# JoeyYoung/adapcc

Hardware: NVIDIA B200
Metric: gpt2_small_ddp_train_tokens_per_sec (higher is better)
Workload: dtype bf16; 1 GPU; model=gpt2-small-double-heads (12L d768 h12 ctx1024 vocab50262, 124476673 params), global_batch=4, per_gpu_batch=4, candidates=2, seq_len=1024, parallelism=dp1, engine=graph, algo=auto, optimizer=adamw+clip1.0 (fused), grad_dtype=bf16, zero_copy_grads=False, buckets=6, zero1=False, lm_rows=all, lm_chunk_rows=8192, relay_control=False

## Files before the change

### adapcc_b200/csrc/ops_norm.cu

```cuda
#include <cuda_bf16.h>

#include <algorithm>

#include "common.h"
#include "device_prims.cuh"

namespace adapcc {

constexpr int kLnWarps = 8;

__device__ __forceinline__ float warp_sum(float v) {
#pragma unroll
  for (int o = 16; o > 0; o >>= 1) v += __shfl_xor_sync(0xffffffffu, v, o);
  return v;
}

template <int VPL, bool RES>
__global__ void __launch_bounds__(kLnWarps * 32, VPL <= 3 ? 3 : 2)
ln_fwd_kernel(const __nv_bfloat16* __restrict__ x, const __nv_bfloat16* __restrict__ res,
              const __nv_bfloat16* __restrict__ gamma, const __nv_bfloat16* __restrict__ beta,
              __nv_bfloat16* __restrict__ sum_out, __nv_bfloat16* __restrict__ y, float* __restrict__ mean,
              float* __restrict__ rstd, int rows, float eps) {
  constexpr int D = VPL * 256;
  const int lane = threadIdx.x & 31, warp = threadIdx.x >> 5;
  uint4 gp[VPL], bp[VPL];
#pragma unroll
  for (int v = 0; v < VPL; ++v) {
    gp[v] = reinterpret_cast<const uint4*>(gamma)[lane + 32 * v];
    bp[v] = reinterpret_cast<const uint4*>(beta)[lane + 32 * v];
  }
  for (int r = blockIdx.x * kLnWarps + warp; r < rows; r += gridDim.x * kLnWarps) {
    const uint4* xr = reinterpret_cast<const uint4*>(x + (size_t)r * D);
    float f[VPL][8];
    float s = 0.f;
#pragma unroll
    for (int v = 0; v < VPL; ++v) {
      unpack<__nv_bfloat16>(ld16(xr + lane + 32 * v), f[v]);
      if constexpr (RES) {
        float fr[8];
        unpack<__nv_bfloat16>(ld16(reinterpret_cast<const uint4*>(res + (size_t)r * D) + lane + 32 * v), fr);
#pragma unroll
        for (int i = 0; i < 8; ++i) f[v][i] += fr[i];
        const uint4 packed = pack<__nv_bfloat16>(f[v]);
        st16(reinterpret_cast<uint4*>(sum_out + (size_t)r * D) + lane + 32 * v, packed);
        unpack<__nv_bfloat16>(packed, f[v]);
      }
#pragma unroll
      for (int i = 0; i < 8; ++i) s += f[v][i];
    }
    const float mu = warp_sum(s) * (1.f / D);
    float q = 0.f;
#pragma unroll
    for (int v = 0; v < VPL; ++v)
#pragma unroll
      for (int i = 0; i < 8; ++i) { const float d = f[v][i] - mu; q += d * d; }
    const float rs = rsqrtf(warp_sum(q) * (1.f / D) + eps);
    uint4* yr = reinterpret_cast<uint4*>(y + (size_t)r * D);
#pragma unroll
    for (int v = 0; v < VPL; ++v) {
      float o[8], g[8], b[8];
      unpack<__nv_bfloat16>(gp[v], g);
      unpack<__nv_bfloat16>(bp[v], b);
#pragma unroll
      for (int i = 0; i < 8; ++i) o[i] = (f[v][i] - mu) * rs * g[i] + b[i];
      st16(yr + lane + 32 * v, pack<__nv_bfloat16>(o));
    }
    if (lane == 0) { mean[r] = mu; rstd[r] = rs; }
  }
}

template <int VPL, bool RES>
__global__ void __launch_bounds__(kLnWarps * 32, VPL <= 3 ? 2 : 1)
ln_bwd_kernel(const __nv_bfloat16* __restrict__ dy, const __nv_bfloat16* __restrict__ x,
              const __nv_bfloat16* __restrict__ gamma, const float* __restrict__ mean, const float* __restrict__ rstd,
              const __nv_bfloat16* __restrict__ dres, __nv_bfloat16* __restrict__ dx,
              float* __restrict__ part_dgamma, float* __restrict__ part_dbeta, int rows) {
  constexpr int D = VPL * 256;
  const int lane = threadIdx.x & 31, warp = threadIdx.x >> 5;
  uint4 gp[VPL];
  float dg[VPL][8], db[VPL][8];
#pragma unroll
  for (int v = 0; v < VPL; ++v) {
    gp[v] = reinterpret_cast<const uint4*>(gamma)[lane + 32 * v];
#pragma unroll
    for (int i = 0; i < 8; ++i) dg[v][i] = db[v][i] = 0.f;
  }
  for (int r = blockIdx.x * kLnWarps + warp; r < rows; r += gridDim.x * kLnWarps) {
    const uint4* xr = reinterpret_cast<const uint4*>(x + (size_t)r * D);
    const uint4* dr = reinterpret_cast<const uint4*>(dy + (size_t)r * D);
    const float mu = mean[r], rs = rstd[r];
    float xh[VPL][8], gy[VPL][8];
    float c1 = 0.f, c2 = 0.f;
#pragma unroll
    for (int v = 0; v < VPL; ++v) {
      float fx[8], fd[8], g[8];
      unpack<__nv_bfloat16>(ld16(xr + lane + 32 * v), fx);
      unpack<__nv_bfloat16>(ld16(dr + lane + 32 * v), fd);
      unpack<__nv_bfloat16>(gp[v], g);
#pragma unroll
      for (int i = 0; i < 8; ++i) {
        xh[v][i] = (fx[i] - mu) * rs;
        gy[v][i] = fd[i] * g[i];
        c1 += gy[v][i];
        c2 += gy[v][i] * xh[v][i];
        dg[v][i] += fd[i] * xh[v][i];
        db[v][i] += fd[i];
      }
    }
    c1 = warp_sum(c1) * (1.f / D);
    c2 = warp_sum(c2) * (1.f / D);
    uint4* ox = reinterpret_cast<uint4*>(dx + (size_t)r * D);
#pragma unroll
    for (int v = 0; v < VPL; ++v) {
      float o[8];
#pragma unroll
      for (int i = 0; i < 8; ++i) o[i] = rs * (gy[v][i] - c1 - xh[v][i] * c2);
      if constexpr (RES) {
        float fr[8];
        unpack<__nv_bfloat16>(ld16(reinterpret_cast<const uint4*>(dres + (size_t)r * D) + lane + 32 * v), fr);
#pragma unroll
        for (int i = 0; i < 8; ++i) o[i] += fr[i];
      }
      st16(ox + lane + 32 * v, pack<__nv_bfloat16>(o));
    }
  }
  __shared__ float sm[kLnWarps][D];
#pragma unroll
  for (int pass = 0; pass < 2; ++pass) {
#pragma unroll
    for (int v = 0; v < VPL; ++v)
#pragma unroll
      for (int i = 0; i < 8; ++i) sm[warp][(lane + 32 * v) * 8 + i] = pass == 0 ? dg[v][i] : db[v][i];
    __syncthreads();
    float* out = (pass == 0 ? part_dgamma : part_dbeta) + (size_t)blockIdx.x * D;
    for (int c = threadIdx.x; c < D; c += blockDim.x) {
      float s = 0.f;
#pragma unroll
      for (int w = 0; w < kLnWarps; ++w) s += sm[w][c];
      out[c] = s;
    }
    __syncthreads();
  }
}

template <typename O>
__global__ void __launch_bounds__(1024)
colsum_finalize_kernel(const float* __restrict__ part, int nparts, int cols, O* __restrict__ out) {
  __shared__ float sm[32][33];
  const int c = blockIdx.x * 32 + threadIdx.x;
  float s = 0.f;
  if (c < cols)
    for (int p = threadIdx.y; p < nparts; p += 32) s += part[(size_t)p * cols + c];
  sm[threadIdx.y][threadIdx.x] = s;
  __syncthreads();
  if (threadIdx.y == 0 && c < cols) {
    float t = 0.f;
#pragma unroll
    for (int r = 0; r < 32; ++r) t += sm[r][threadIdx.x];
    out[c] = from_float<O>(t);
  }
}

template <typename O>
__global__ void __launch_bounds__(1024)
colsum_finalize_pair_kernel(const float* __restrict__ part_a, const float* __restrict__ part_b, int nparts, int cols,
                            O* __restrict__ out_a, O* __restrict__ out_b) {
  __shared__ float sm[32][33];
  const float* part = blockIdx.y == 0 ? part_a : part_b;
  O* out = blockIdx.y == 0 ? out_a : out_b;
  const int c = blockIdx.x * 32 + threadIdx.x;
  float s = 0.f;
  if (c < cols)
    for (int p = threadIdx.y; p < nparts; p += 32) s += part[(size_t)p * cols + c];
  sm[threadIdx.y][threadIdx.x] = s;
  __syncthreads();
  if (threadIdx.y == 0 && c < cols) {
    float t = 0.f;
#pragma unroll
    for (int r = 0; r < 32; ++r) t += sm[r][threadIdx.x];
    out[c] = from_float<O>(t);
  }
}

__global__ void __launch_bounds__(256)
colsum_partial_kernel(const __nv_bfloat16* __restrict__ a, int rows, int cols, float* __restrict__ part) {
  const int vcol = blockIdx.x * 32 + threadIdx.x;
  const int nvec = cols / 8;
  float acc[8];
#pragma unroll
  for (int i = 0; i < 8; ++i) acc[i] = 0.f;
  if (vcol < nvec) {
    for (int r = blockIdx.y * 8 + threadIdx.y; r < rows; r += gridDim.y * 8) {
      float f[8];
      unpack<__nv_bfloat16>(ld16(reinterpret_cast<const uint4*>(a + (size_t)r * cols) + vcol), f);
#pragma unroll
      for (int i = 0; i < 8; ++i) acc[i] += f[i];
    }
  }
  __shared__ float sm[8][32][8];
#pragma unroll
  for (int i = 0; i < 8; ++i) sm[threadIdx.y][threadIdx.x][i] = acc[i];
  __syncthreads();
  if (threadIdx.y == 0 && vcol < nvec) {
#pragma unroll
    for (int i = 0; i < 8; ++i) {
      float s = 0.f;
#pragma unroll
      for (int w = 0; w < 8; ++w) s += sm[w][threadIdx.x][i];
      part[(size_t)blockIdx.y * cols + vcol * 8 + i] = s;
    }
  }
}

}

using namespace adapcc;

extern "C" {

static int ln_grid(int rows, int per_sm) {
  const int groups = std::max(1, (rows + kLnWarps - 1) / kLnWarps);
  const int cap = 148 * per_sm;
  const int iters = (groups + cap - 1) / cap;
  return (groups + iters - 1) / iters;
}
static int ln_fwd_ctas_per_sm(int d) { return d <= 768 ? 3 : 2; }
static int ln_bwd_ctas_per_sm(int d) { return d <= 768 ? 2 : 1; }
int adapcc_ln_partials(int rows) { return ln_grid(rows, 2); }

static int ln_fwd_launch(const void* x, const void* res, const void* gamma, const void* beta, void* sum_out, void* y,
                         float* mean, float* rstd, int rows, int d, float eps, void* stream) {
  cudaStream_t s = (cudaStream_t)stream;
  if (rows <= 0) return 0;
  const int grid = ln_grid(rows, ln_fwd_ctas_per_sm(d));
#define LN_FWD(V)                                                                                                  \
  do {                                                                                                             \
    if (res)                                                                                                       \
      ln_fwd_kernel<V, true><<<grid, kLnWarps * 32, 0, s>>>((const __nv_bfloat16*)x, (const __nv_bfloat16*)res,    \
          (const __nv_bfloat16*)gamma, (const __nv_bfloat16*)beta, (__nv_bfloat16*)sum_out, (__nv_bfloat16*)y,     \
          mean, rstd, rows, eps);                                                                                  \
    else                                                                                                           \
      ln_fwd_kernel<V, false><<<grid, kLnWarps * 32, 0, s>>>((const __nv_bfloat16*)x, nullptr,                     \
          (const __nv_bfloat16*)gamma, (const __nv_bfloat16*)beta, nullptr, (__nv_bfloat16*)y, mean, rstd, rows,   \
          eps);                                                                                                    \
  } while (0)
  switch (d) {
    case 256: LN_FWD(1); break;
    case 512: LN_FWD(2); break;
    case 768: LN_FWD(3); break;
    case 1024: LN_FWD(4); break;
    default: set_error("ln_fwd: unsupported width %d (256/512/768/1024)", d); return -1;
  }
#undef LN_FWD
  CUDA_TRY(cudaGetLastError());
  count_launch();
  return 0;
}

int adapcc_ln_fwd(const void* x, const void* gamma, const void* beta, void* y, float* mean, float* rstd, int rows,
                  int d, float eps, void* stream) {
  return ln_fwd_launch(x, nullptr, gamma, beta, nullptr, y, mean, rstd, rows, d, eps, stream);
}

int adapcc_add_ln_fwd(const void* x, const void* res, const void* gamma, const void* beta, void* sum_out, void* y,
                      float* mean, float* rstd, int rows, int d, float eps, void* stream) {
  if (!res || !sum_out) { set_error("add_ln_fwd: res and sum_out are required"); return -1; }
  return ln_fwd_launch(x, res, gamma, beta, sum_out, y, mean, rstd, rows, d, eps, stream);
}

static int ln_bwd_launch(const void* dy, const void* x, const void* gamma, const float* mean, const float* rstd,
                         const void* dres, void* dx, void* dgamma, void* dbeta, float* part, int rows, int d,
                         void* stream) {
  cudaStream_t s = (cudaStream_t)stream;
  if (rows <= 0) return 0;
  const int grid = ln_grid(rows, ln_bwd_ctas_per_sm(d));
  float* pg = part;
  float* pb = part + (size_t)grid * d;
#define LN_BWD(V)                                                                                                  \
  do {                                                                                                             \
    if (dres)                                                                                                      \
      ln_bwd_kernel<V, true><<<grid, kLnWarps * 32, 0, s>>>((const __nv_bfloat16*)dy, (const __nv_bfloat16*)x,     \
          (const __nv_bfloat16*)gamma, mean, rstd, (const __nv_bfloat16*)dres, (__nv_bfloat16*)dx, pg, pb, rows);  \
    else                                                                                                           \
      ln_bwd_kernel<V, false><<<grid, kLnWarps * 32, 0, s>>>((const __nv_bfloat16*)dy, (const __nv_bfloat16*)x,    \
          (const __nv_bfloat16*)gamma, mean, rstd, nullptr, (__nv_bfloat16*)dx, pg, pb, rows);                     \
  } while (0)
  switch (d) {
    case 256: LN_BWD(1); break;
    case 512: LN_BWD(2); break;
    case 768: LN_BWD(3); break;
    case 1024: LN_BWD(4); break;
    default: set_error("ln_bwd: unsupported width %d (256/512/768/1024)", d); return -1;
  }
#undef LN_BWD
  CUDA_TRY(cudaGetLastError());
  colsum_finalize_pair_kernel<__nv_bfloat16><<<dim3((d + 31) / 32, 2), dim3(32, 32), 0, s>>>(
      pg, pb, grid, d, (__nv_bfloat16*)dgamma, (__nv_bfloat16*)dbeta);
  CUDA_TRY(cudaGetLastError());
  count_launch(2);
  return 0;
}

int adapcc_ln_bwd(const void* dy, const void* x, const void* gamma, const float* mean, const float* rstd, void* dx,
                  void* dgamma, void* dbeta, float* part, int rows, int d, void* stream) {
  return ln_bwd_launch(dy, x, gamma, mean, rstd, nullptr, dx, dgamma, dbeta, part, rows, d, stream);
}

int adapcc_add_ln_bwd(const void* dy, const void* x, const void* gamma, const float* mean, const float* rstd,
                      const void* dres, void* dx, void* dgamma, void* dbeta, float* part, int rows, int d,
                      void* stream) {
  return ln_bwd_launch(dy, x, gamma, mean, rstd, dres, dx, dgamma, dbeta, part, rows, d, stream);
}

int adapcc_colsum_splits(int rows) { return std::max(1, std::min(64, rows / 64)); }

int adapcc_colsum(const void* a, int rows, int cols, void* out, float* part, void* stream) {
  cudaStream_t s = (cudaStream_t)stream;
  if (cols % 8 != 0) { set_error("colsum: cols must be a multiple of 8"); return -1; }
  if (rows <= 0) return 0;
  const int splits = adapcc_colsum_splits(rows);
  dim3 grid((cols / 8 + 31) / 32, splits), block(32, 8);
  colsum_partial_kernel<<<grid, block, 0, s>>>((const __nv_bfloat16*)a, rows, cols, part);
  colsum_finalize_kernel<__nv_bfloat16><<<(cols + 31) / 32, dim3(32, 32), 0, s>>>(part, splits, cols, (__nv_bfloat16*)out);
  CUDA_TRY(cudaGetLastError());
  count_launch(2);
  return 0;
}

}
```

### adapcc_b200/models/gpt2.py

```python
from __future__ import annotations

import math
import os
from dataclasses import dataclass
from typing import Optional, Tuple

import torch
import torch.nn as nn
import torch.nn.functional as F

from ..ops.layers import FusedLayerNorm, FusedLinear


@dataclass
class GPT2Config:

    vocab_size: int = 50257 + 5
    n_positions: int = 1024
    n_embd: int = 768
    n_layer: int = 12
    n_head: int = 12
    layer_norm_epsilon: float = 1e-5
    initializer_range: float = 0.02
    lm_chunk_rows: int = 8192

    @classmethod
    def tiny(cls) -> "GPT2Config":
        return cls(vocab_size=512, n_positions=64, n_embd=64, n_layer=2, n_head=4, lm_chunk_rows=64)


class Block(nn.Module):

    def __init__(self, cfg: GPT2Config):
        super().__init__()
        d = cfg.n_embd
        self.n_head = cfg.n_head
        self.ln_1 = FusedLayerNorm(d, eps=cfg.layer_norm_epsilon)
        self.c_attn = FusedLinear(d, 3 * d)
        self.c_proj = FusedLinear(d, d)
        self.ln_2 = FusedLayerNorm(d, eps=cfg.layer_norm_epsilon)
        self.c_fc = FusedLinear(d, 4 * d)
        self.c_proj2 = FusedLinear(4 * d, d)
        self.tc_mlp = int(os.environ.get("ADAPCC_TCGEN05_MLP", "2") or 0)

    def _mlp(self, h: torch.Tensor) -> torch.Tensor:
        if self.tc_mlp and h.is_cuda and h.dtype == torch.bfloat16 and torch.is_grad_enabled():
            from ..ops.gemm import linear_gelu, mlp_gelu, supported
            if supported(h, self.c_fc.weight):
                if self.tc_mlp >= 2 and self.c_fc.weight.shape[0] % 64 == 0:
                    return mlp_gelu(h, self.c_fc.weight, self.c_fc.bias, self.c_proj2.weight, self.c_proj2.bias)
                return self.c_proj2(linear_gelu(h, self.c_fc.weight, self.c_fc.bias))
        return self.c_proj2(F.gelu(self.c_fc(h), approximate="tanh"))

    def _attn(self, h: torch.Tensor) -> torch.Tensor:
        B, T, D = h.shape
        q, k, v = (t.view(B, T, self.n_head, D // self.n_head).transpose(1, 2) for t in self.c_attn(h).split(D, dim=-1))
        a = F.scaled_dot_product_attention(q, k, v, is_causal=True)
        return self.c_proj(a.transpose(1, 2).reshape(B, T, D))

    def forward_deferred(self, x: torch.Tensor, delta: Optional[torch.Tensor]):
        if delta is None:
            h = self.ln_1(x)
        else:
            x, h = self.ln_1.forward_add(x, delta)
        x, h = self.ln_2.forward_add(x, self._attn(h))
        return x, self._mlp(h)

    def forward(self, x: torch.Tensor) -> torch.Tensor:
        x = x + self._attn(self.ln_1(x))
        return x + self._mlp(self.ln_2(x))


def use_sink(p) -> bool:
    from ..ops.layers import _sink
    return p.is_cuda and _sink(p) is not None


class _ChunkedLMLoss(torch.autograd.Function):

    @staticmethod
    def forward(ctx, h, weight, labels, chunk, vocab, scale=None):
        n = h.shape[0]
        use_kernel = h.is_cuda and h.dtype == torch.bfloat16 and weight.shape[0] % 8 == 0
        grad_h = torch.empty_like(h)
        grad_w = None
        total = torch.zeros((), dtype=torch.float32, device=h.device)
        direct = False
        if use_kernel:
            from ..ops import fused_ce_
            from ..ops.layers import _sink
            direct = (scale is not None and _sink(weight) is not None and weight.grad.dtype == h.dtype
                      and ctx.needs_input_grad[1])
        for s in range(0, n, chunk):
            hs = h[s:s + chunk]
            ls = labels[s:s + chunk]
            logits = hs @ weight.t()
            if use_kernel:
                total += fused_ce_(logits, ls, vocab, grad_scale=scale).sum()
                g = logits
            else:
                lf = logits.float()
                lf[:, vocab:] = float("-inf")
                valid = (ls >= 0)
                lse = torch.logsumexp(lf, dim=-1)
                tgt = lf.gather(1, ls.clamp(min=0).unsqueeze(1)).squeeze(1)
                total += ((lse - tgt) * valid).sum()
                p = torch.softmax(lf, dim=-1)
                p.scatter_add_(1, ls.clamp(min=0).unsqueeze(1), -torch.ones_like(p[:, :1]))
                g = p * valid.unsqueeze(1)
                if scale is not None:
                    g = g * scale
                g = g.to(h.dtype)
            torch.mm(g, weight, out=grad_h[s:s + chunk])
            if direct:
                if s == 0:
                    torch.mm(g.t(), hs, out=weight.grad)
                else:
                    weight.grad.addmm_(g.t(), hs)
            elif grad_w is None:
                grad_w = g.t() @ hs
            else:
                grad_w.addmm_(g.t(), hs)
        if scale is not None:
            total = total * scale.reshape(())
        ctx.direct, ctx.weight = direct, weight
        if direct:
            ctx.save_for_backward(grad_h)
        else:
            if grad_w is None:
                grad_w = torch.zeros_like(weight)
            ctx.save_for_backward(grad_h, grad_w)
        return total

    @staticmethod
    def backward(ctx, g):
        if ctx.direct:
            return ctx.saved_tensors[0], None, None, None, None, None
        grad_h, grad_w = ctx.saved_tensors
        gw = grad_w * g.to(grad_w.dtype)
        if use_sink(ctx.weight):
            ctx.weight.grad.add_(gw)
            gw = None
        return grad_h * g.to(grad_h.dtype), gw, None, None, None, None


class GPT2DoubleHeads(nn.Module):

    def __init__(self, cfg: Optional[GPT2Config] = None):
        super().__init__()
        self.cfg = cfg = cfg or GPT2Config()
        self.padded_vocab = (cfg.vocab_size + 63) // 64 * 64
        self.wte = nn.Embedding(self.padded_vocab, cfg.n_embd)
        self.wpe = nn.Embedding(cfg.n_positions, cfg.n_embd)
        self.h = nn.ModuleList([Block(cfg) for _ in range(cfg.n_layer)])
        self.ln_f = FusedLayerNorm(cfg.n_embd, eps=cfg.layer_norm_epsilon)
        self.mc_head = nn.Linear(cfg.n_embd, 1)
        self.lm_row_capacity = 0
        self.fuse_add_ln = os.environ.get("ADAPCC_FUSE_ADD_LN", "1") == "1"
        self.fused_embed = os.environ.get("ADAPCC_FUSED_EMBED", "1") != "0"
        if self.fused_embed:
            self.wte.weight._adapcc_embed_table = True
            self.wpe.weight._adapcc_embed_table = True
        self._pos_cache = {}
        self.apply(self._init)
        for blk in self.h:
            for lin in (blk.c_proj, blk.c_proj2):
                nn.init.normal_(lin.weight, std=cfg.initializer_range / math.sqrt(2 * cfg.n_layer))

    def _init(self, m):
        if isinstance(m, (nn.Linear, nn.Embedding)):
            nn.init.normal_(m.weight, std=self.cfg.initializer_range)
            if isinstance(m, nn.Linear) and m.bias is not None:
                nn.init.zeros_(m.bias)

    def num_parameters(self) -> int:
        return sum(p.numel() for p in self.parameters())

    def hidden(self, input_ids: torch.Tensor, token_type_ids: Optional[torch.Tensor]) -> torch.Tensor:
        N, T = input_ids.shape
        if (self.fused_embed and input_ids.is_cuda and self.wte.weight.dtype == torch.bfloat16
                and self.wpe.weight.dtype == torch.bfloat16):
            from ..ops import fused_embedding_sum
            key = (N, T, input_ids.device)
            pos = self._pos_cache.get(key)
            if pos is None:
                pos = self._pos_cache[key] = torch.arange(T, device=input_ids.device).repeat(N)
            lookups = [(0, input_ids), (1, pos)] + ([(0, token_type_ids)] if token_type_ids is not None else [])
            x = fused_embedding_sum([self.wte.weight, self.wpe.weight], lookups).view(N, T, -1)
        else:
            pos = torch.arange(T, device=input_ids.device)
            x = self.wte(input_ids) + self.wpe(pos)[None]
            if token_type_ids is not None:
                x = x + self.wte(token_type_ids)
        if self.fuse_add_ln:
            delta = None
            for blk in self.h:
                x, delta = blk.forward_deferred(x, delta)
            return self.ln_f.forward_add(x, delta)[1]
        for blk in self.h:
            x = blk(x)
        return self.ln_f(x)

    def forward(self, input_ids, token_type_ids=None, mc_token_ids=None, lm_labels=None, mc_labels=None,
                lm_coef: float = 1.0, mc_coef: float = 1.0) -> Tuple[torch.Tensor, torch.Tensor, torch.Tensor]:
        B, C, T = input_ids.shape
        ids = input_ids.reshape(B * C, T)
        tt = token_type_ids.reshape(B * C, T) if token_type_ids is not None else None
        h = self.hidden(ids, tt)
        zero = torch.zeros((), dtype=torch.float32, device=h.device)
        lm_loss, mc_loss = zero, zero
        if lm_labels is not None:
            labels = lm_labels.reshape(B * C, T)
            shift_h = h[:, :-1].reshape(-1, h.shape[-1])
            shift_l = labels[:, 1:].reshape(-1)
            n_valid = (shift_l >= 0).sum()
            cap = int(self.lm_row_capacity)
            compact = 0 < cap < shift_l.numel()
            if compact:
                order = torch.argsort((shift_l < 0).to(torch.int8), stable=True)[:cap]
                shift_h = shift_h.index_select(0, order)
                shift_l = shift_l.index_select(0, order)
            scale = (lm_coef / n_valid.clamp(min=1).to(torch.float32)).reshape(1)
            lm_term = _ChunkedLMLoss.apply(shift_h, self.wte.weight, shift_l, self.cfg.lm_chunk_rows,
                                           self.cfg.vocab_size, scale)
            lm_loss = lm_term / lm_coef if lm_coef != 0 else lm_term
            if compact:
                lm_loss = torch.where(n_valid > cap, torch.full_like(lm_loss, float("nan")), lm_loss)
                lm_term = torch.where(n_valid > cap, torch.full_like(lm_term, float("nan")), lm_term)
        if mc_token_ids is not None and mc_labels is not None:
            idx = mc_token_ids.reshape(B * C, 1, 1).expand(-1, 1, h.shape[-1])
            cls_h = h.gather(1, idx).squeeze(1)
            mc_logits = self.mc_head(cls_h).view(B, C).float()
            mc_loss = F.cross_entropy(mc_logits, mc_labels)
        loss = (lm_term if lm_labels is not None else zero) + mc_coef * mc_loss
        return loss, lm_loss, mc_loss


@torch.no_grad()
def sample_sequence(model: "GPT2DoubleHeads", input_ids: torch.Tensor, token_type_ids: Optional[torch.Tensor] = None,
                    max_new_tokens: int = 20, temperature: float = 0.7, top_k: int = 0, top_p: float = 0.9,
                    eos_token: Optional[int] = None, reply_type: Optional[int] = None,
                    generator: Optional[torch.Generator] = None) -> torch.Tensor:
    ids = input_ids.clone()
    tt = token_type_ids.clone() if token_type_ids is not None else None
    vocab = model.cfg.vocab_size
    for _ in range(max_new_tokens):
        window = slice(max(0, ids.shape[1] - model.cfg.n_positions), None)
        h = model.hidden(ids[:, window], tt[:, window] if tt is not None else None)
        logits = (h[:, -1].float() @ model.wte.weight.float().t())[:, :vocab] / max(temperature, 1e-6)
        if top_k > 0:
            kth = torch.topk(logits, min(top_k, vocab)).values[:, -1:]
            logits = logits.masked_fill(logits < kth, float("-inf"))
        if 0.0 < top_p < 1.0:
            srt, idx = torch.sort(logits, descending=True)
            cum = torch.softmax(srt, -1).cumsum(-1)
            drop = cum > top_p
            drop[:, 1:] = drop[:, :-1].clone()
            drop[:, 0] = False
            logits = logits.masked_fill(torch.zeros_like(drop).scatter(1, idx, drop), float("-inf"))
        nxt = torch.multinomial(torch.softmax(logits, -1), 1, generator=generator)
        ids = torch.cat([ids, nxt], 1)
        if tt is not None:
            tt = torch.cat([tt, torch.full_like(nxt, reply_type if reply_type is not None else int(tt[0, -1]))], 1)
        if eos_token is not None and int(nxt) == eos_token:
            break
    return ids[:, input_ids.shape[1]:]


def lm_rows_needed(lm_labels: torch.Tensor, multiple: int = 256) -> int:
    n = int((lm_labels[..., 1:] >= 0).sum())
    return max(multiple, (n + multiple - 1) // multiple * multiple)


def synthetic_batch(batch: int, candidates: int, seq_len: int, vocab: int, device="cpu", seed: int = 0,
                    pin: bool = False):
    g = torch.Generator().manual_seed(seed)
    ids = torch.randint(0, vocab, (batch, candidates, seq_len), generator=g)
    tt = torch.randint(vocab - 5, vocab - 3, (batch, candidates, seq_len), generator=g)
    labels = torch.full((batch, candidates, seq_len), -100, dtype=torch.long)
    reply = max(1, seq_len // 4)
    labels[:, -1, -reply:] = ids[:, -1, -reply:]
    mc_token_ids = torch.full((batch, candidates), seq_len - 1, dtype=torch.long)
    mc_labels = torch.full((batch,), candidates - 1, dtype=torch.long)
    out = {"input_ids": ids, "token_type_ids": tt, "lm_labels": labels, "mc_token_ids": mc_token_ids,
           "mc_labels": mc_labels}
    if pin and torch.cuda.is_available():
        out = {k: v.pin_memory() for k, v in out.items()}
    if device != "cpu":
        out = {k: v.to(device, non_blocking=True) for k, v in out.items()}
    return out
```

### adapcc_b200/ops/gemm.py

```python
from __future__ import annotations

import os
from ctypes import c_int, c_void_p
from typing import Optional, Tuple

import torch

from ..runtime.native import NativeError, last_error, load_library

_bound = False
ACT = {"none": 0, "gelu": 1, "dgelu": 2, "residual": 3}


def _lib():
    global _bound
    lib = load_library()
    if not _bound:
        lib.adapcc_gemm_bias_act_v.argtypes = [c_void_p] * 5 + [c_int] * 5 + [c_void_p]
        lib.adapcc_gemm_pp.argtypes = [c_void_p] * 6 + [c_int] * 4 + [c_void_p]
        _bound = True
    return lib


def supported(x: torch.Tensor, weight: torch.Tensor) -> bool:
    return (x.is_cuda and x.dtype == torch.bfloat16 and weight.dtype == torch.bfloat16
            and weight.shape[1] % 64 == 0 and weight.shape[0] % 128 == 0)


def default_variant() -> int:
    return int(os.environ.get("ADAPCC_TCGEN05_VARIANT", "3"))


def linear_act(x: torch.Tensor, weight: torch.Tensor, bias: Optional[torch.Tensor], act: str = "gelu",
               save_pre: bool = False, variant: Optional[int] = None,
               aux: Optional[torch.Tensor] = None,
               colsum: Optional[torch.Tensor] = None) -> Tuple[torch.Tensor, Optional[torch.Tensor]]:
    if not supported(x, weight):
        raise NativeError("linear_act: needs bf16 CUDA tensors with K % 64 == 0 and N % 128 == 0")
    n, k = weight.shape
    x2 = x.reshape(-1, k).contiguous()
    w = weight.contiguous()
    m = x2.shape[0]
    code = ACT[act]
    out = torch.empty(m, n, dtype=torch.bfloat16, device=x.device)
    v_req = default_variant() if variant is None else int(variant)
    if v_req == 3 and n % 256 == 0 and code <= 2:
        if code == 2:
            if aux is None or aux.numel() != m * n or aux.dtype != torch.bfloat16:
                raise NativeError("linear_act(dgelu): aux must be a bf16 tensor with the result's shape")
            pre = aux.reshape(m, n).contiguous()
        else:
            pre = torch.empty_like(out) if save_pre else None
        if colsum is not None and (code != 2 or colsum.dtype != torch.float32 or colsum.numel() != n):
            raise NativeError("linear_act: colsum is an fp32 [N] accumulator of the dgelu mode")
        b = bias.contiguous() if bias is not None else None
        rc = _lib().adapcc_gemm_pp(c_void_p(x2.data_ptr()), c_void_p(w.data_ptr()),
                                   c_void_p(b.data_ptr() if b is not None else 0), c_void_p(out.data_ptr()),
                                   c_void_p(pre.data_ptr() if pre is not None else 0),
                                   c_void_p(colsum.data_ptr() if colsum is not None else 0), m, n, k, code,
                                   c_void_p(torch.cuda.current_stream().cuda_stream))
        if rc != 0:
            raise NativeError(f"gemm_pp failed: {last_error()}")
        shape = x.shape[:-1] + (n,)
        return out.view(shape), (pre.view(shape) if (pre is not None and code < 2) else None)
    if colsum is not None:
        raise NativeError("linear_act: colsum needs variant 3 (N % 256 == 0)")
    if v_req == 3:
        v_req = 1
    if code >= 2:
        if aux is None or aux.numel() != m * n or aux.dtype != torch.bfloat16:
            raise NativeError(f"linear_act({act}): aux must be a bf16 tensor with the result's shape")
        pre = aux.reshape(m, n).contiguous()
        v = 0
    else:
        pre = torch.empty_like(out) if save_pre else None
        v = v_req
    b = bias.contiguous() if bias is not None else None
    rc = _lib().adapcc_gemm_bias_act_v(c_void_p(x2.data_ptr()), c_void_p(w.data_ptr()),
                                       c_void_p(b.data_ptr() if b is not None else 0), c_void_p(out.data_ptr()),
                                       c_void_p(pre.data_ptr() if pre is not None else 0), m, n, k, code, v,
                                       c_void_p(torch.cuda.current_stream().cuda_stream))
    if rc != 0:
        raise NativeError(f"gemm_bias_act failed: {last_error()}")
    shape = x.shape[:-1] + (n,)
    return out.view(shape), (pre.view(shape) if (pre is not None and code < 2) else None)


class _LinearGeluFn(torch.autograd.Function):
    @staticmethod
    def forward(ctx, x, w, b):
        out, pre = linear_act(x, w, b, "gelu", save_pre=True)
        ctx.save_for_backward(x, w, pre)
        ctx.params = (w, b)
        return out

    @staticmethod
    def backward(ctx, dy):
        from .layers import linear_backward
        x, w, pre = ctx.saved_tensors
        du = torch.ops.aten.gelu_backward(dy.contiguous(), pre, approximate="tanh")
        return linear_backward(ctx.params, x, w, du, ctx.needs_input_grad[0])


def linear_gelu(x: torch.Tensor, weight: torch.Tensor, bias: torch.Tensor) -> torch.Tensor:
    return _LinearGeluFn.apply(x, weight, bias)


class _MLPFn(torch.autograd.Function):

    @staticmethod
    def forward(ctx, x, w1, b1, w2, b2):
        h, pre = linear_act(x, w1, b1, "gelu", save_pre=True)
        y = torch.nn.functional.linear(h, w2, b2)
        ctx.save_for_backward(x, w1, w2, pre, h)
        ctx.params = ((w1, b1), (w2, b2))
        return y

    @staticmethod
    def backward(ctx, dy):
        from .layers import linear_backward
        x, w1, w2, pre, h = ctx.saved_tensors
        p1, p2 = ctx.params
        dy = dy.contiguous()
        _, dw2, db2 = linear_backward(p2, h, w2, dy, needs_dx=False)
        w2t = w2.t().contiguous()
        if default_variant() == 3 and w2t.shape[0] % 256 == 0:
            db_acc = torch.zeros(w2t.shape[0], dtype=torch.float32, device=dy.device)
            du, _ = linear_act(dy, w2t, None, "dgelu", aux=pre, colsum=db_acc, variant=3)
            dx, dw1, db1 = linear_backward(p1, x, w1, du, ctx.needs_input_grad[0], db=db_acc)
        else:
            du, _ = linear_act(dy, w2t, None, "dgelu", aux=pre)
            dx, dw1, db1 = linear_backward(p1, x, w1, du, ctx.needs_input_grad[0])
        return dx, dw1, db1, dw2, db2


def mlp_gelu(x, w1, b1, w2, b2):
    return _MLPFn.apply(x, w1, b1, w2, b2)
```

### adapcc_b200/ops/layers.py

```python
from __future__ import annotations

from ctypes import c_float, c_int, c_void_p

import torch
import torch.nn as nn
import torch.nn.functional as F

from ..runtime.native import NativeError, last_error, load_library

_bound = False
_LN_WIDTHS = (256, 512, 768, 1024)


def _lib():
    global _bound
    lib = load_library()
    if not _bound:
        lib.adapcc_ln_fwd.argtypes = [c_void_p, c_void_p, c_void_p, c_void_p, c_void_p, c_void_p, c_int, c_int,
                                      c_float, c_void_p]
        lib.adapcc_ln_bwd.argtypes = [c_void_p] * 9 + [c_int, c_int, c_void_p]
        lib.adapcc_add_ln_fwd.argtypes = [c_void_p] * 8 + [c_int, c_int, c_float, c_void_p]
        lib.adapcc_add_ln_bwd.argtypes = [c_void_p] * 10 + [c_int, c_int, c_void_p]
        lib.adapcc_ln_partials.argtypes = [c_int]
        lib.adapcc_colsum.argtypes = [c_void_p, c_int, c_int, c_void_p, c_void_p, c_void_p]
        lib.adapcc_colsum_splits.argtypes = [c_int]
        _bound = True
    return lib


def _s():
    return c_void_p(torch.cuda.current_stream().cuda_stream)


def _p(t):
    return c_void_p(t.data_ptr())


def _sink(p):
    if p is None or p.grad is None:
        return None
    return getattr(p, "_adapcc_grad_sink", None)


class _LayerNormFn(torch.autograd.Function):
    @staticmethod
    def forward(ctx, x, gamma, beta, eps):
        lib = _lib()
        d = x.shape[-1]
        x2 = x.reshape(-1, d).contiguous()
        rows = x2.shape[0]
        y = torch.empty_like(x2)
        mean = torch.empty(rows, dtype=torch.float32, device=x.device)
        rstd = torch.empty(rows, dtype=torch.float32, device=x.device)
        if lib.adapcc_ln_fwd(_p(x2), _p(gamma), _p(beta), _p(y), _p(mean), _p(rstd), rows, d, eps, _s()) != 0:
            raise NativeError(f"ln_fwd failed: {last_error()}")
        ctx.save_for_backward(x2, gamma, mean, rstd)
        ctx.params = (gamma, beta)
        return y.view(x.shape)

    @staticmethod
    def backward(ctx, dy):
        lib = _lib()
        x2, gamma, mean, rstd = ctx.saved_tensors
        rows, d = x2.shape
        dy2 = dy.reshape(rows, d).contiguous()
        dx = torch.empty_like(x2)
        dgamma, dbeta, finish = _ln_param_grads(ctx.params)
        part = torch.empty(2 * lib.adapcc_ln_partials(rows) * d, dtype=torch.float32, device=x2.device)
        if lib.adapcc_ln_bwd(_p(dy2), _p(x2), _p(gamma), _p(mean), _p(rstd), _p(dx), _p(dgamma), _p(dbeta), _p(part),
                             rows, d, _s()) != 0:
            raise NativeError(f"ln_bwd failed: {last_error()}")
        return (dx.view(dy.shape),) + finish() + (None,)


def _ln_param_grads(params):
    gamma, beta = params
    sg, sb = _sink(gamma), _sink(beta)
    dgamma = gamma.grad if sg is not None and sg.begin() else torch.empty_like(gamma)
    dbeta = beta.grad if sb is not None and sb.begin() else torch.empty_like(beta)

    def finish():
        if sg is not None:
            sg.done()
        if sb is not None:
            sb.done()
        return (None if sg is not None else dgamma, None if sb is not None else dbeta)
    return dgamma, dbeta, finish


class _AddLayerNormFn(torch.autograd.Function):

    @staticmethod
    def forward(ctx, x, res, gamma, beta, eps):
        lib = _lib()
        d = x.shape[-1]
        x2 = x.reshape(-1, d).contiguous()
        r2 = res.reshape(-1, d).contiguous()
        rows = x2.shape[0]
        ssum = torch.empty_like(x2)
        y = torch.empty_like(x2)
        mean = torch.empty(rows, dtype=torch.float32, device=x.device)
        rstd = torch.empty(rows, dtype=torch.float32, device=x.device)
        if lib.adapcc_add_ln_fwd(_p(x2), _p(r2), _p(gamma), _p(beta), _p(ssum), _p(y), _p(mean), _p(rstd), rows, d,
                                 eps, _s()) != 0:
            raise NativeError(f"add_ln_fwd failed: {last_error()}")
        ctx.save_for_backward(ssum, gamma, mean, rstd)
        ctx.params = (gamma, beta)
        ctx.set_materialize_grads(False)
        return ssum.view(x.shape), y.view(x.shape)

    @staticmethod
    def backward(ctx, dsum, dy):
        lib = _lib()
        s2, gamma, mean, rstd = ctx.saved_tensors
        rows, d = s2.shape
        if dy is None:
            return dsum, dsum, None, None, None
        dy2 = dy.reshape(rows, d).contiguous()
        ds2 = None if dsum is None else dsum.reshape(rows, d).contiguous()
        dx = torch.empty_like(s2)
        dgamma, dbeta, finish = _ln_param_grads(ctx.params)
        part = torch.empty(2 * lib.adapcc_ln_partials(rows) * d, dtype=torch.float32, device=s2.device)
        if lib.adapcc_add_ln_bwd(_p(dy2), _p(s2), _p(gamma), _p(mean), _p(rstd), c_void_p(0) if ds2 is None else _p(ds2),
                                 _p(dx), _p(dgamma), _p(dbeta), _p(part), rows, d, _s()) != 0:
            raise NativeError(f"add_ln_bwd failed: {last_error()}")
        dx = dx.view(dy.shape)
        return (dx, dx) + finish() + (None,)


class FusedLayerNorm(nn.LayerNorm):

    def _fusable(self, x):
        return (x.is_cuda and x.dtype == torch.bfloat16 and self.weight.dtype == torch.bfloat16
                and x.shape[-1] in _LN_WIDTHS and len(self.normalized_shape) == 1)

    def forward(self, x):
        if self._fusable(x):
            return _LayerNormFn.apply(x, self.weight, self.bias, self.eps)
        return F.layer_norm(x, self.normalized_shape, self.weight, self.bias, self.eps)

    def forward_add(self, x, res):
        if self._fusable(x) and res.shape == x.shape and res.dtype == x.dtype:
            return _AddLayerNormFn.apply(x, res, self.weight, self.bias, self.eps)
        s = x + res
        return s, F.layer_norm(s, self.normalized_shape, self.weight, self.bias, self.eps)


class _LinearFn(torch.autograd.Function):
    @staticmethod
    def forward(ctx, x, w, b):
        ctx.save_for_backward(x, w)
        ctx.params = (w, b)
        return F.linear(x, w, b)

    @staticmethod
    def backward(ctx, dy):
        x, w = ctx.saved_tensors
        return linear_backward(ctx.params, x, w, dy, ctx.needs_input_grad[0])


def linear_backward(params, x, w, dy, needs_dx=True, db=None):
    lib = _lib()
    n = w.shape[0]
    dy2 = dy.reshape(-1, n)
    if not dy2.is_contiguous():
        dy2 = dy2.contiguous()
    x2 = x.reshape(-1, x.shape[-1])
    dx = (dy2 @ w).view(x.shape) if needs_dx else None
    pw, pb = params
    sw, sb = _sink(pw), _sink(pb)
    if sw is not None and sw.begin():
        torch.mm(dy2.t(), x2, out=pw.grad)
        sw.done()
        dw = None
    else:
        dw = dy2.t() @ x2
    rows = dy2.shape[0]
    direct_b = sb is not None and pb.grad.dtype == dy2.dtype and sb.begin()
    if db is not None:
        if direct_b:
            pb.grad.copy_(db)
            sb.done()
            return dx, dw, None
        return dx, dw, db.to(dy2.dtype)
    db = pb.grad if direct_b else torch.empty(n, dtype=dy2.dtype, device=dy2.device)
    part = torch.empty(lib.adapcc_colsum_splits(rows) * n, dtype=torch.float32, device=dy2.device)
    if lib.adapcc_colsum(_p(dy2), rows, n, _p(db), _p(part), _s()) != 0:
        raise NativeError(f"colsum failed: {last_error()}")
    if direct_b:
        sb.done()
    return dx, dw, None if direct_b else db


class FusedLinear(nn.Linear):

    def forward(self, x):
        if (x.is_cuda and x.dtype == torch.bfloat16 and self.bias is not None and self.weight.dtype == torch.bfloat16
                and self.out_features % 8 == 0 and torch.is_grad_enabled()):
            return _LinearFn.apply(x, self.weight, self.bias)
        return F.linear(x, self.weight, self.bias)
```

Measured before the change: 940,400 tokens/s.

## Fold linear bias gradients into layernorm backward and QKV pack kernels

Adds a bias-gradient handoff so that the column sum for the attention-projection and MLP output biases is computed inside the add+layernorm backward kernel, and the QKV bias gradient inside a new kernel that packs dq/dk/dv into the qkv gradient layout. This removes separate colsum passes and the contiguous copy for the QKV split backward. It also rewrites the layernorm forward and backward kernels to use non-caching vector loads and shared-memory float4 accumulators for the parameter partials. The cost is extra autograd plumbing that matches on pointer identity, and wider per-block partial buffers.

```diff
diff --git a/adapcc_b200/csrc/ops_norm.cu b/adapcc_b200/csrc/ops_norm.cu
--- a/adapcc_b200/csrc/ops_norm.cu
+++ b/adapcc_b200/csrc/ops_norm.cu
@@ -8,10 +8,24 @@
 namespace adapcc {
 
 constexpr int kLnWarps = 8;
+constexpr int kLnRows = 1;
 
 __device__ __forceinline__ float warp_sum(float v) {
 #pragma unroll
   for (int o = 16; o > 0; o >>= 1) v += __shfl_xor_sync(0xffffffffu, v, o);
+  return v;
+}
+
+__device__ __forceinline__ uint4 ldg16(const void* p) {
+  uint4 v;
+  asm("ld.global.nc.L1::no_allocate.v4.u32 {%0,%1,%2,%3}, [%4];"
+      : "=r"(v.x), "=r"(v.y), "=r"(v.z), "=r"(v.w) : "l"(p));
+  return v;
+}
+__device__ __forceinline__ void stg16(void* p, uint4 v) { *reinterpret_cast<uint4*>(p) = v; }
+__device__ __forceinline__ uint4 opaque(uint4 v) {
+  asm volatile("mov.b32 %0, %0;\n\tmov.b32 %1, %1;\n\tmov.b32 %2, %2;\n\tmov.b32 %3, %3;"
+               : "+r"(v.x), "+r"(v.y), "+r"(v.z), "+r"(v.w));
   return v;
 }
 
@@ -21,125 +35,209 @@
               const __nv_bfloat16* __restrict__ gamma, const __nv_bfloat16* __restrict__ beta,
               __nv_bfloat16* __restrict__ sum_out, __nv_bfloat16* __restrict__ y, float* __restrict__ mean,
               float* __restrict__ rstd, int rows, float eps) {
-  constexpr int D = VPL * 256;
+  constexpr int D = VPL * 256, R = kLnRows;
   const int lane = threadIdx.x & 31, warp = threadIdx.x >> 5;
-  uint4 gp[VPL], bp[VPL];
-#pragma unroll
-  for (int v = 0; v < VPL; ++v) {
-    gp[v] = reinterpret_cast<const uint4*>(gamma)[lane + 32 * v];
-    bp[v] = reinterpret_cast<const uint4*>(beta)[lane + 32 * v];
-  }
-  for (int r = blockIdx.x * kLnWarps + warp; r < rows; r += gridDim.x * kLnWarps) {
-    const uint4* xr = reinterpret_cast<const uint4*>(x + (size_t)r * D);
-    float f[VPL][8];
-    float s = 0.f;
-#pragma unroll
-    for (int v = 0; v < VPL; ++v) {
-      unpack<__nv_bfloat16>(ld16(xr + lane + 32 * v), f[v]);
-      if constexpr (RES) {
-        float fr[8];
-        unpack<__nv_bfloat16>(ld16(reinterpret_cast<const uint4*>(res + (size_t)r * D) + lane + 32 * v), fr);
-#pragma unroll
-        for (int i = 0; i < 8; ++i) f[v][i] += fr[i];
-        const uint4 packed = pack<__nv_bfloat16>(f[v]);
-        st16(reinterpret_cast<uint4*>(sum_out + (size_t)r * D) + lane + 32 * v, packed);
-        unpack<__nv_bfloat16>(packed, f[v]);
-      }
-#pragma unroll
-      for (int i = 0; i < 8; ++i) s += f[v][i];
-    }
-    const float mu = warp_sum(s) * (1.f / D);
-    float q = 0.f;
-#pragma unroll
-    for (int v = 0; v < VPL; ++v)
-#pragma unroll
-      for (int i = 0; i < 8; ++i) { const float d = f[v][i] - mu; q += d * d; }
-    const float rs = rsqrtf(warp_sum(q) * (1.f / D) + eps);
-    uint4* yr = reinterpret_cast<uint4*>(y + (size_t)r * D);
-#pragma unroll
-    for (int v = 0; v < VPL; ++v) {
-      float o[8], g[8], b[8];
-      unpack<__nv_bfloat16>(gp[v], g);
-      unpack<__nv_bfloat16>(bp[v], b);
-#pragma unroll
-      for (int i = 0; i < 8; ++i) o[i] = (f[v][i] - mu) * rs * g[i] + b[i];
-      st16(yr + lane + 32 * v, pack<__nv_bfloat16>(o));
-    }
-    if (lane == 0) { mean[r] = mu; rstd[r] = rs; }
-  }
-}
-
-template <int VPL, bool RES>
+  const uint4* g4 = reinterpret_cast<const uint4*>(gamma);
+  const uint4* b4 = reinterpret_cast<const uint4*>(beta);
+  for (int r0 = (blockIdx.x * kLnWarps + warp) * R; r0 < rows; r0 += gridDim.x * kLnWarps * R) {
+    int row[R];
+    uint4 p[R][VPL], q[R][VPL];
+#pragma unroll
+    for (int j = 0; j < R; ++j) {
+      row[j] = min(r0 + j, rows - 1);
+#pragma unroll
+      for (int v = 0; v < VPL; ++v) {
+        p[j][v] = ldg16(x + (size_t)row[j] * D + (lane + 32 * v) * 8);
+        if constexpr (RES) q[j][v] = ldg16(res + (size_t)row[j] * D + (lane + 32 * v) * 8);
+      }
+    }
+    float s[R];
+#pragma unroll
+    for (int j = 0; j < R; ++j) {
+      s[j] = 0.f;
+#pragma unroll
+      for (int v = 0; v < VPL; ++v) {
+        float f[8];
+        unpack<__nv_bfloat16>(p[j][v], f);
+        if constexpr (RES) {
+          float fr[8];
+          unpack<__nv_bfloat16>(q[j][v], fr);
+#pragma unroll
+          for (int i = 0; i < 8; ++i) f[i] += fr[i];
+          p[j][v] = pack<__nv_bfloat16>(f);
+          if (r0 + j < rows) stg16(sum_out + (size_t)row[j] * D + (lane + 32 * v) * 8, p[j][v]);
+          unpack<__nv_bfloat16>(p[j][v], f);
+        }
+#pragma unroll
+        for (int i = 0; i < 8; ++i) s[j] += f[i];
+      }
+    }
+    float mu[R], rs[R];
+#pragma unroll
+    for (int j = 0; j < R; ++j) mu[j] = warp_sum(s[j]) * (1.f / D);
+#pragma unroll
+    for (int j = 0; j < R; ++j) {
+      s[j] = 0.f;
+#pragma unroll
+      for (int v = 0; v < VPL; ++v) {
+        float f[8];
+        unpack<__nv_bfloat16>(opaque(p[j][v]), f);
+#pragma unroll
+        for (int i = 0; i < 8; ++i) { const float d = f[i] - mu[j]; s[j] += d * d; }
+      }
+    }
+#pragma unroll
+    for (int j = 0; j < R; ++j) rs[j] = rsqrtf(warp_sum(s[j]) * (1.f / D) + eps);
+#pragma unroll
+    for (int j = 0; j < R; ++j) {
+      if (r0 + j >= rows) break;
+#pragma unroll
+      for (int v = 0; v < VPL; ++v) {
+        float f[8], o[8], g[8], b[8];
+        unpack<__nv_bfloat16>(opaque(p[j][v]), f);
+        unpack<__nv_bfloat16>(__ldg(g4 + lane + 32 * v), g);
+        unpack<__nv_bfloat16>(__ldg(b4 + lane + 32 * v), b);
+#pragma unroll
+        for (int i = 0; i < 8; ++i) o[i] = (f[i] - mu[j]) * rs[j] * g[i] + b[i];
+        stg16(y + (size_t)row[j] * D + (lane + 32 * v) * 8, pack<__nv_bfloat16>(o));
+      }
+      if (lane == 0) { mean[row[j]] = mu[j]; rstd[row[j]] = rs[j]; }
+    }
+  }
+}
+
+constexpr int ln_bwd_smem(int vpl, int nsum) { return kLnWarps * nsum * vpl * 2 * 32 * 16; }
+
+template <int VPL, bool RES, bool BIAS>
 __global__ void __launch_bounds__(kLnWarps * 32, VPL <= 3 ? 2 : 1)
 ln_bwd_kernel(const __nv_bfloat16* __restrict__ dy, const __nv_bfloat16* __restrict__ x,
               const __nv_bfloat16* __restrict__ gamma, const float* __restrict__ mean, const float* __restrict__ rstd,
-              const __nv_bfloat16* __restrict__ dres, __nv_bfloat16* __restrict__ dx,
-              float* __restrict__ part_dgamma, float* __restrict__ part_dbeta, int rows) {
-  constexpr int D = VPL * 256;
+              const __nv_bfloat16* __restrict__ dres, __nv_bfloat16* __restrict__ dx, float* __restrict__ part,
+              int rows) {
+  constexpr int D = VPL * 256, R = kLnRows, NSUM = BIAS ? 3 : 2, SLOTS = NSUM * VPL * 2 * 32;
   const int lane = threadIdx.x & 31, warp = threadIdx.x >> 5;
-  uint4 gp[VPL];
-  float dg[VPL][8], db[VPL][8];
-#pragma unroll
-  for (int v = 0; v < VPL; ++v) {
-    gp[v] = reinterpret_cast<const uint4*>(gamma)[lane + 32 * v];
-#pragma unroll
-    for (int i = 0; i < 8; ++i) dg[v][i] = db[v][i] = 0.f;
-  }
-  for (int r = blockIdx.x * kLnWarps + warp; r < rows; r += gridDim.x * kLnWarps) {
-    const uint4* xr = reinterpret_cast<const uint4*>(x + (size_t)r * D);
-    const uint4* dr = reinterpret_cast<const uint4*>(dy + (size_t)r * D);
-    const float mu = mean[r], rs = rstd[r];
-    float xh[VPL][8], gy[VPL][8];
-    float c1 = 0.f, c2 = 0.f;
+  extern __shared__ float4 acc_all[];
+  float4* acc = acc_all + warp * SLOTS + lane;
+#pragma unroll
+  for (int k = 0; k < SLOTS / 32; ++k) acc[k * 32] = make_float4(0.f, 0.f, 0.f, 0.f);
+  const uint4* g4 = reinterpret_cast<const uint4*>(gamma);
+  for (int r0 = (blockIdx.x * kLnWarps + warp) * R; r0 < rows; r0 += gridDim.x * kLnWarps * R) {
+    int row[R];
+    float mu[R], rs[R];
+    uint4 px[R][VPL], pd[R][VPL], pr[R][VPL];
+#pragma unroll
+    for (int j = 0; j < R; ++j) {
+      row[j] = min(r0 + j, rows - 1);
+      mu[j] = mean[row[j]];
+      rs[j] = rstd[row[j]];
+#pragma unroll
+      for (int v = 0; v < VPL; ++v) {
+        px[j][v] = ldg16(x + (size_t)row[j] * D + (lane + 32 * v) * 8);
+        pd[j][v] = ldg16(dy + (size_t)row[j] * D + (lane + 32 * v) * 8);
+        if constexpr (RES) pr[j][v] = ldg16(dres + (size_t)row[j] * D + (lane + 32 * v) * 8);
+      }
+    }
+    float c1[R], c2[R];
+#pragma unroll
+    for (int j = 0; j < R; ++j) {
+      c1[j] = c2[j] = 0.f;
+#pragma unroll
+      for (int v = 0; v < VPL; ++v) {
+        float fx[8], fd[8], g[8];
+        unpack<__nv_bfloat16>(px[j][v], fx);
+        unpack<__nv_bfloat16>(pd[j][v], fd);
+        unpack<__nv_bfloat16>(__ldg(g4 + lane + 32 * v), g);
+#pragma unroll
+        for (int i = 0; i < 8; ++i) {
+          const float gy = fd[i] * g[i];
+          c1[j] += gy;
+          c2[j] += gy * ((fx[i] - mu[j]) * rs[j]);
+        }
+      }
+    }
+#pragma unroll
+    for (int j = 0; j < R; ++j) {
+      c1[j] = warp_sum(c1[j]) * (1.f / D);
+      c2[j] = warp_sum(c2[j]) * (1.f / D);
+    }
 #pragma unroll
     for (int v = 0; v < VPL; ++v) {
-      float fx[8], fd[8], g[8];
-      unpack<__nv_bfloat16>(ld16(xr + lane + 32 * v), fx);
-      unpack<__nv_bfloat16>(ld16(dr + lane + 32 * v), fd);
-      unpack<__nv_bfloat16>(gp[v], g);
-#pragma unroll
-      for (int i = 0; i < 8; ++i) {
-        xh[v][i] = (fx[i] - mu) * rs;
-        gy[v][i] = fd[i] * g[i];
-        c1 += gy[v][i];
-        c2 += gy[v][i] * xh[v][i];
-        dg[v][i] += fd[i] * xh[v][i];
-        db[v][i] += fd[i];
-      }
-    }
-    c1 = warp_sum(c1) * (1.f / D);
-    c2 = warp_sum(c2) * (1.f / D);
-    uint4* ox = reinterpret_cast<uint4*>(dx + (size_t)r * D);
-#pragma unroll
-    for (int v = 0; v < VPL; ++v) {
-      float o[8];
-#pragma unroll
-      for (int i = 0; i < 8; ++i) o[i] = rs * (gy[v][i] - c1 - xh[v][i] * c2);
-      if constexpr (RES) {
-        float fr[8];
-        unpack<__nv_bfloat16>(ld16(reinterpret_cast<const uint4*>(dres + (size_t)r * D) + lane + 32 * v), fr);
-#pragma unroll
-        for (int i = 0; i < 8; ++i) o[i] += fr[i];
-      }
-      st16(ox + lane + 32 * v, pack<__nv_bfloat16>(o));
-    }
-  }
-  __shared__ float sm[kLnWarps][D];
-#pragma unroll
-  for (int pass = 0; pass < 2; ++pass) {
-#pragma unroll
-    for (int v = 0; v < VPL; ++v)
-#pragma unroll
-      for (int i = 0; i < 8; ++i) sm[warp][(lane + 32 * v) * 8 + i] = pass == 0 ? dg[v][i] : db[v][i];
-    __syncthreads();
-    float* out = (pass == 0 ? part_dgamma : part_dbeta) + (size_t)blockIdx.x * D;
-    for (int c = threadIdx.x; c < D; c += blockDim.x) {
-      float s = 0.f;
-#pragma unroll
-      for (int w = 0; w < kLnWarps; ++w) s += sm[w][c];
-      out[c] = s;
-    }
-    __syncthreads();
+      float g[8], sg[8], sb[8], sx[8];
+      unpack<__nv_bfloat16>(__ldg(g4 + lane + 32 * v), g);
+#pragma unroll
+      for (int i = 0; i < 8; ++i) sg[i] = sb[i] = sx[i] = 0.f;
+#pragma unroll
+      for (int j = 0; j < R; ++j) {
+        if (r0 + j >= rows) break;
+        float fx[8], fd[8], o[8];
+        unpack<__nv_bfloat16>(opaque(px[j][v]), fx);
+        unpack<__nv_bfloat16>(opaque(pd[j][v]), fd);
+#pragma unroll
+        for (int i = 0; i < 8; ++i) {
+          const float xh = (fx[i] - mu[j]) * rs[j];
+          o[i] = rs[j] * (fd[i] * g[i] - c1[j] - xh * c2[j]);
+          sg[i] += fd[i] * xh;
+          sb[i] += fd[i];
+        }
+        if constexpr (RES) {
+          float fr[8];
+          unpack<__nv_bfloat16>(pr[j][v], fr);
+#pragma unroll
+          for (int i = 0; i < 8; ++i) o[i] += fr[i];
+        }
+        const uint4 packed = pack<__nv_bfloat16>(o);
+        stg16(dx + (size_t)row[j] * D + (lane + 32 * v) * 8, packed);
+        if constexpr (BIAS) {
+          unpack<__nv_bfloat16>(packed, o);
+#pragma unroll
+          for (int i = 0; i < 8; ++i) sx[i] += o[i];
+        }
+      }
+#pragma unroll
+      for (int k = 0; k < NSUM; ++k) {
+        const float* src = k == 0 ? sg : k == 1 ? sb : sx;
+#pragma unroll
+        for (int h = 0; h < 2; ++h) {
+          float4& a = acc[((k * VPL + v) * 2 + h) * 32];
+          a.x += src[4 * h]; a.y += src[4 * h + 1]; a.z += src[4 * h + 2]; a.w += src[4 * h + 3];
+        }
+      }
+    }
+  }
+  __syncthreads();
+  for (int s = threadIdx.x; s < SLOTS; s += blockDim.x) {
+    float4 t = acc_all[s];
+#pragma unroll
+    for (int w = 1; w < kLnWarps; ++w) {
+      const float4 u = acc_all[w * SLOTS + s];
+      t.x += u.x; t.y += u.y; t.z += u.z; t.w += u.w;
+    }
+    const int l = s & 31, h = (s >> 5) & 1, v = (s >> 6) % VPL, k = (s >> 6) / VPL;
+    const int c = (l + 32 * v) * 8 + 4 * h;
+    *reinterpret_cast<float4*>(part + ((size_t)k * gridDim.x + blockIdx.x) * D + c) = t;
+  }
+}
+
+__global__ void __launch_bounds__(1024)
+ln_param_finalize_kernel(const float* __restrict__ part, int nparts, int cols, __nv_bfloat16* __restrict__ dgamma,
+                         __nv_bfloat16* __restrict__ dbeta, void* __restrict__ dbias, int dbias_fp32) {
+  __shared__ float sm[32][33];
+  const int k = blockIdx.y;
+  const float* pk = part + (size_t)k * nparts * cols;
+  const int c = blockIdx.x * 32 + threadIdx.x;
+  float s = 0.f;
+  if (c < cols)
+    for (int p = threadIdx.y; p < nparts; p += 32) s += pk[(size_t)p * cols + c];
+  sm[threadIdx.y][threadIdx.x] = s;
+  __syncthreads();
+  if (threadIdx.y == 0 && c < cols) {
+    float t = 0.f;
+#pragma unroll
+    for (int r = 0; r < 32; ++r) t += sm[r][threadIdx.x];
+    if (k == 0) dgamma[c] = __float2bfloat16_rn(t);
+    else if (k == 1) dbeta[c] = __float2bfloat16_rn(t);
+    else if (dbias_fp32) static_cast<float*>(dbias)[c] = t;
+    else static_cast<__nv_bfloat16*>(dbias)[c] = __float2bfloat16_rn(t);
   }
 }
 
@@ -161,24 +259,48 @@
   }
 }
 
-template <typename O>
-__global__ void __launch_bounds__(1024)
-colsum_finalize_pair_kernel(const float* __restrict__ part_a, const float* __restrict__ part_b, int nparts, int cols,
-                            O* __restrict__ out_a, O* __restrict__ out_b) {
-  __shared__ float sm[32][33];
-  const float* part = blockIdx.y == 0 ? part_a : part_b;
-  O* out = blockIdx.y == 0 ? out_a : out_b;
-  const int c = blockIdx.x * 32 + threadIdx.x;
-  float s = 0.f;
-  if (c < cols)
-    for (int p = threadIdx.y; p < nparts; p += 32) s += part[(size_t)p * cols + c];
-  sm[threadIdx.y][threadIdx.x] = s;
+struct QkvSrc {
+  const __nv_bfloat16* p[3];
+  long long sb[3], sh[3], st[3];
+};
+
+__global__ void __launch_bounds__(256)
+qkv_pack_colsum_kernel(QkvSrc src, int T, int hd, int D, int rows, __nv_bfloat16* __restrict__ out,
+                       float* __restrict__ part) {
+  const int cols = 3 * D;
+  const int vcol = blockIdx.x * 32 + threadIdx.x;
+  float acc[8];
+#pragma unroll
+  for (int i = 0; i < 8; ++i) acc[i] = 0.f;
+  if (vcol < cols / 8) {
+    const int j = vcol * 8 / D, w = vcol * 8 - j * D, h = w / hd, e = w - h * hd;
+    const __nv_bfloat16* base = (j == 0 ? src.p[0] : j == 1 ? src.p[1] : src.p[2]) +
+                                h * (j == 0 ? src.sh[0] : j == 1 ? src.sh[1] : src.sh[2]) + e;
+    const long long sb = j == 0 ? src.sb[0] : j == 1 ? src.sb[1] : src.sb[2];
+    const long long st = j == 0 ? src.st[0] : j == 1 ? src.st[1] : src.st[2];
+#pragma unroll 4
+    for (int r = blockIdx.y * 8 + threadIdx.y; r < rows; r += gridDim.y * 8) {
+      const int b = r / T, t = r - b * T;
+      const uint4 v = ldg16(base + b * sb + t * st);
+      stg16(out + (size_t)r * cols + vcol * 8, v);
+      float f[8];
+      unpack<__nv_bfloat16>(v, f);
+#pragma unroll
+      for (int i = 0; i < 8; ++i) acc[i] += f[i];
+    }
+  }
+  __shared__ float sm[8][32][8];
+#pragma unroll
+  for (int i = 0; i < 8; ++i) sm[threadIdx.y][threadIdx.x][i] = acc[i];
   __syncthreads();
-  if (threadIdx.y == 0 && c < cols) {
-    float t = 0.f;
-#pragma unroll
-    for (int r = 0; r < 32; ++r) t += sm[r][threadIdx.x];
-    out[c] = from_float<O>(t);
+  if (threadIdx.y == 0 && vcol < cols / 8) {
+#pragma unroll
+    for (int i = 0; i < 8; ++i) {
+      float s = 0.f;
+#pragma unroll
+      for (int w = 0; w < 8; ++w) s += sm[w][threadIdx.x][i];
+      part[(size_t)blockIdx.y * cols + vcol * 8 + i] = s;
+    }
   }
 }
 
@@ -219,7 +341,7 @@
 extern "C" {
 
 static int ln_grid(int rows, int per_sm) {
-  const int groups = std::max(1, (rows + kLnWarps - 1) / kLnWarps);
+  const int groups = std::max(1, (rows + kLnWarps * kLnRows - 1) / (kLnWarps * kLnRows));
   const int cap = 148 * per_sm;
   const int iters = (groups + cap - 1) / cap;
   return (groups + iters - 1) / iters;
@@ -268,34 +390,58 @@
   return ln_fwd_launch(x, res, gamma, beta, sum_out, y, mean, rstd, rows, d, eps, stream);
 }
 
+int adapcc_colsum_splits(int rows) { return std::max(1, std::min(64, rows / 64)); }
+
+}
+
+template <int VPL, bool RES, bool BIAS>
+static cudaError_t ln_bwd_variant(int grid, cudaStream_t s, const void* dy, const void* x, const void* gamma,
+                                  const float* mean, const float* rstd, const void* dres, void* dx, float* part,
+                                  int rows) {
+  constexpr int smem = ln_bwd_smem(VPL, BIAS ? 3 : 2);
+  static bool configured = false;
+  if (!configured) {
+    const cudaError_t e = cudaFuncSetAttribute(ln_bwd_kernel<VPL, RES, BIAS>,
+                                               cudaFuncAttributeMaxDynamicSharedMemorySize, smem);
+    if (e != cudaSuccess) return e;
+    configured = true;
+  }
+  ln_bwd_kernel<VPL, RES, BIAS><<<grid, kLnWarps * 32, smem, s>>>((const __nv_bfloat16*)dy, (const __nv_bfloat16*)x,
+      (const __nv_bfloat16*)gamma, mean, rstd, (const __nv_bfloat16*)dres, (__nv_bfloat16*)dx, part, rows);
+  return cudaGetLastError();
+}
+
+template <int VPL>
+static cudaError_t ln_bwd_dispatch(bool res, bool bias, int grid, cudaStream_t s, const void* dy, const void* x,
+                                   const void* gamma, const float* mean, const float* rstd, const void* dres, void* dx,
+                                   float* part, int rows) {
+  if (res)
+    return bias ? ln_bwd_variant<VPL, true, true>(grid, s, dy, x, gamma, mean, rstd, dres, dx, part, rows)
+                : ln_bwd_variant<VPL, true, false>(grid, s, dy, x, gamma, mean, rstd, dres, dx, part, rows);
+  return bias ? ln_bwd_variant<VPL, false, true>(grid, s, dy, x, gamma, mean, rstd, dres, dx, part, rows)
+              : ln_bwd_variant<VPL, false, false>(grid, s, dy, x, gamma, mean, rstd, dres, dx, part, rows);
+}
+
+extern "C" {
+
 static int ln_bwd_launch(const void* dy, const void* x, const void* gamma, const float* mean, const float* rstd,
-                         const void* dres, void* dx, void* dgamma, void* dbeta, float* part, int rows, int d,
-                         void* stream) {
+                         const void* dres, void* dx, void* dgamma, void* dbeta, void* dbias, int dbias_fp32,
+                         float* part, int rows, int d, void* stream) {
   cudaStream_t s = (cudaStream_t)stream;
   if (rows <= 0) return 0;
   const int grid = ln_grid(rows, ln_bwd_ctas_per_sm(d));
-  float* pg = part;
-  float* pb = part + (size_t)grid * d;
-#define LN_BWD(V)                                                                                                  \
-  do {                                                                                                             \
-    if (dres)                                                                                                      \
-      ln_bwd_kernel<V, true><<<grid, kLnWarps * 32, 0, s>>>((const __nv_bfloat16*)dy, (const __nv_bfloat16*)x,     \
-          (const __nv_bfloat16*)gamma, mean, rstd, (const __nv_bfloat16*)dres, (__nv_bfloat16*)dx, pg, pb, rows);  \
-    else                                                                                                           \
-      ln_bwd_kernel<V, false><<<grid, kLnWarps * 32, 0, s>>>((const __nv_bfloat16*)dy, (const __nv_bfloat16*)x,    \
-          (const __nv_bfloat16*)gamma, mean, rstd, nullptr, (__nv_bfloat16*)dx, pg, pb, rows);                     \
-  } while (0)
+  const bool res = dres != nullptr, bias = dbias != nullptr;
+  cudaError_t e;
   switch (d) {
-    case 256: LN_BWD(1); break;
-    case 512: LN_BWD(2); break;
-    case 768: LN_BWD(3); break;
-    case 1024: LN_BWD(4); break;
+    case 256: e = ln_bwd_dispatch<1>(res, bias, grid, s, dy, x, gamma, mean, rstd, dres, dx, part, rows); break;
+    case 512: e = ln_bwd_dispatch<2>(res, bias, grid, s, dy, x, gamma, mean, rstd, dres, dx, part, rows); break;
+    case 768: e = ln_bwd_dispatch<3>(res, bias, grid, s, dy, x, gamma, mean, rstd, dres, dx, part, rows); break;
+    case 1024: e = ln_bwd_dispatch<4>(res, bias, grid, s, dy, x, gamma, mean, rstd, dres, dx, part, rows); break;
     default: set_error("ln_bwd: unsupported width %d (256/512/768/1024)", d); return -1;
   }
-#undef LN_BWD
-  CUDA_TRY(cudaGetLastError());
-  colsum_finalize_pair_kernel<__nv_bfloat16><<<dim3((d + 31) / 32, 2), dim3(32, 32), 0, s>>>(
-      pg, pb, grid, d, (__nv_bfloat16*)dgamma, (__nv_bfloat16*)dbeta);
+  CUDA_TRY(e);
+  ln_param_finalize_kernel<<<dim3((d + 31) / 32, bias ? 3 : 2), dim3(32, 32), 0, s>>>(
+      part, grid, d, (__nv_bfloat16*)dgamma, (__nv_bfloat16*)dbeta, dbias, dbias_fp32);
   CUDA_TRY(cudaGetLastError());
   count_launch(2);
   return 0;
@@ -303,16 +449,52 @@
 
 int adapcc_ln_bwd(const void* dy, const void* x, const void* gamma, const float* mean, const float* rstd, void* dx,
                   void* dgamma, void* dbeta, float* part, int rows, int d, void* stream) {
-  return ln_bwd_launch(dy, x, gamma, mean, rstd, nullptr, dx, dgamma, dbeta, part, rows, d, stream);
+  return ln_bwd_launch(dy, x, gamma, mean, rstd, nullptr, dx, dgamma, dbeta, nullptr, 0, part, rows, d, stream);
 }
 
 int adapcc_add_ln_bwd(const void* dy, const void* x, const void* gamma, const float* mean, const float* rstd,
                       const void* dres, void* dx, void* dgamma, void* dbeta, float* part, int rows, int d,
                       void* stream) {
-  return ln_bwd_launch(dy, x, gamma, mean, rstd, dres, dx, dgamma, dbeta, part, rows, d, stream);
-}
-
-int adapcc_colsum_splits(int rows) { return std::max(1, std::min(64, rows / 64)); }
+  return ln_bwd_launch(dy, x, gamma, mean, rstd, dres, dx, dgamma, dbeta, nullptr, 0, part, rows, d, stream);
+}
+
+int adapcc_add_ln_bwd_bias(const void* dy, const void* x, const void* gamma, const float* mean, const float* rstd,
+                           const void* dres, void* dx, void* dgamma, void* dbeta, void* dbias, int dbias_fp32,
+                           float* part, int rows, int d, void* stream) {
+  if (!dbias) { set_error("add_ln_bwd_bias: dbias is required"); return -1; }
+  return ln_bwd_launch(dy, x, gamma, mean, rstd, dres, dx, dgamma, dbeta, dbias, dbias_fp32, part, rows, d, stream);
+}
+
+int adapcc_qkv_pack_colsum(const void* dq, const void* dk, const void* dv, const long long* strides, int B, int H,
+                           int T, int hd, void* dqkv, void* dbias, int dbias_fp32, float* part, void* stream) {
+  cudaStream_t s = (cudaStream_t)stream;
+  QkvSrc src;
+  const void* p[3] = {dq, dk, dv};
+  for (int j = 0; j < 3; ++j) {
+    src.p[j] = (const __nv_bfloat16*)p[j];
+    src.sb[j] = strides[3 * j];
+    src.sh[j] = strides[3 * j + 1];
+    src.st[j] = strides[3 * j + 2];
+    if (((uintptr_t)p[j] & 15) || src.sb[j] % 8 || src.sh[j] % 8 || src.st[j] % 8) {
+      set_error("qkv_pack_colsum: tensor %d needs 16-byte aligned rows (strides multiples of 8 elements)", j);
+      return -1;
+    }
+  }
+  if (hd % 8 != 0) { set_error("qkv_pack_colsum: head dim %d is not a multiple of 8", hd); return -1; }
+  const int rows = B * T, d = H * hd, cols = 3 * d;
+  if (rows <= 0) return 0;
+  const int splits = adapcc_colsum_splits(rows);
+  qkv_pack_colsum_kernel<<<dim3((cols / 8 + 31) / 32, splits), dim3(32, 8), 0, s>>>(src, T, hd, d, rows,
+                                                                                  (__nv_bfloat16*)dqkv, part);
+  if (dbias_fp32)
+    colsum_finalize_kernel<float><<<(cols + 31) / 32, dim3(32, 32), 0, s>>>(part, splits, cols, (float*)dbias);
+  else
+    colsum_finalize_kernel<__nv_bfloat16><<<(cols + 31) / 32, dim3(32, 32), 0, s>>>(part, splits, cols,
+                                                                                    (__nv_bfloat16*)dbias);
+  CUDA_TRY(cudaGetLastError());
+  count_launch(2);
+  return 0;
+}
 
 int adapcc_colsum(const void* a, int rows, int cols, void* out, float* part, void* stream) {
   cudaStream_t s = (cudaStream_t)stream;
diff --git a/adapcc_b200/csrc/ops_transpose.cu b/adapcc_b200/csrc/ops_transpose.cu
--- /dev/null
+++ b/adapcc_b200/csrc/ops_transpose.cu
@@ -0,0 +1,53 @@
+#include <cuda_bf16.h>
+
+#include "common.h"
+
+namespace adapcc {
+
+constexpr int kTile = 64;
+
+__global__ void __launch_bounds__(256)
+transpose_bf16_kernel(const __nv_bfloat16* __restrict__ in, int rows, int cols, __nv_bfloat16* __restrict__ out) {
+  __shared__ __nv_bfloat16 tile[kTile][kTile + 2];
+  const int r0 = blockIdx.y * kTile, c0 = blockIdx.x * kTile;
+  const int tx = threadIdx.x, ty = threadIdx.y;
+#pragma unroll
+  for (int k = 0; k < kTile / 8; ++k) {
+    const int r = r0 + ty + 8 * k, c = c0 + 2 * tx;
+    if (r < rows && c < cols)
+      *reinterpret_cast<__nv_bfloat162*>(&tile[ty + 8 * k][2 * tx]) =
+          *reinterpret_cast<const __nv_bfloat162*>(in + (size_t)r * cols + c);
+  }
+  __syncthreads();
+#pragma unroll
+  for (int k = 0; k < kTile / 8; ++k) {
+    const int c = c0 + ty + 8 * k, r = r0 + 2 * tx;
+    if (c >= cols || r >= rows) continue;
+    __nv_bfloat162 v;
+    v.x = tile[2 * tx][ty + 8 * k];
+    v.y = tile[2 * tx + 1][ty + 8 * k];
+    *reinterpret_cast<__nv_bfloat162*>(out + (size_t)c * rows + r) = v;
+  }
+}
+
+}
+
+using namespace adapcc;
+
+extern "C" {
+
+int adapcc_transpose_bf16(const void* in, int rows, int cols, void* out, void* stream) {
+  if (rows % 2 != 0 || cols % 2 != 0) {
+    set_error("transpose_bf16: rows (%d) and cols (%d) must be even", rows, cols);
+    return -1;
+  }
+  if (rows <= 0 || cols <= 0) return 0;
+  dim3 grid((cols + kTile - 1) / kTile, (rows + kTile - 1) / kTile);
+  transpose_bf16_kernel<<<grid, dim3(32, 8), 0, (cudaStream_t)stream>>>((const __nv_bfloat16*)in, rows, cols,
+                                                                         (__nv_bfloat16*)out);
+  CUDA_TRY(cudaGetLastError());
+  count_launch();
+  return 0;
+}
+
+}
diff --git a/adapcc_b200/models/gpt2.py b/adapcc_b200/models/gpt2.py
--- a/adapcc_b200/models/gpt2.py
+++ b/adapcc_b200/models/gpt2.py
@@ -9,7 +9,7 @@
 import torch.nn as nn
 import torch.nn.functional as F
 
-from ..ops.layers import FusedLayerNorm, FusedLinear
+from ..ops.layers import FusedLayerNorm, FusedLinear, split_heads
 
 
 @dataclass
@@ -42,6 +42,7 @@
         self.c_fc = FusedLinear(d, 4 * d)
         self.c_proj2 = FusedLinear(4 * d, d)
         self.tc_mlp = int(os.environ.get("ADAPCC_TCGEN05_MLP", "2") or 0)
+        self.fold_bias_grad = fold_bias_grad_enabled()
 
     def _mlp(self, h: torch.Tensor) -> torch.Tensor:
         if self.tc_mlp and h.is_cuda and h.dtype == torch.bfloat16 and torch.is_grad_enabled():
@@ -54,21 +55,25 @@
 
     def _attn(self, h: torch.Tensor) -> torch.Tensor:
         B, T, D = h.shape
-        q, k, v = (t.view(B, T, self.n_head, D // self.n_head).transpose(1, 2) for t in self.c_attn(h).split(D, dim=-1))
+        q, k, v = split_heads(self.c_attn(h), self.n_head, self.c_attn.bias if self.fold_bias_grad else None)
         a = F.scaled_dot_product_attention(q, k, v, is_causal=True)
         return self.c_proj(a.transpose(1, 2).reshape(B, T, D))
 
-    def forward_deferred(self, x: torch.Tensor, delta: Optional[torch.Tensor]):
+    def forward_deferred(self, x: torch.Tensor, delta: Optional[torch.Tensor], delta_bias=None):
         if delta is None:
             h = self.ln_1(x)
         else:
-            x, h = self.ln_1.forward_add(x, delta)
-        x, h = self.ln_2.forward_add(x, self._attn(h))
+            x, h = self.ln_1.forward_add(x, delta, res_bias=delta_bias if self.fold_bias_grad else None)
+        x, h = self.ln_2.forward_add(x, self._attn(h), res_bias=self.c_proj.bias if self.fold_bias_grad else None)
         return x, self._mlp(h)
 
     def forward(self, x: torch.Tensor) -> torch.Tensor:
         x = x + self._attn(self.ln_1(x))
         return x + self._mlp(self.ln_2(x))
+
+
+def fold_bias_grad_enabled() -> bool:
+    return os.environ.get("ADAPCC_FOLD_BIAS_GRAD", "1") != "0"
 
 
 def use_sink(p) -> bool:
@@ -157,6 +162,7 @@
         self.mc_head = nn.Linear(cfg.n_embd, 1)
         self.lm_row_capacity = 0
         self.fuse_add_ln = os.environ.get("ADAPCC_FUSE_ADD_LN", "1") == "1"
+        self.fold_bias_grad = fold_bias_grad_enabled()
         self.fused_embed = os.environ.get("ADAPCC_FUSED_EMBED", "1") != "0"
         if self.fused_embed:
             self.wte.weight._adapcc_embed_table = True
@@ -193,10 +199,11 @@
             if token_type_ids is not None:
                 x = x + self.wte(token_type_ids)
         if self.fuse_add_ln:
-            delta = None
+            delta = delta_bias = None
             for blk in self.h:
-                x, delta = blk.forward_deferred(x, delta)
-            return self.ln_f.forward_add(x, delta)[1]
+                x, delta = blk.forward_deferred(x, delta, delta_bias)
+                delta_bias = blk.c_proj2.bias
+            return self.ln_f.forward_add(x, delta, res_bias=delta_bias if self.fold_bias_grad else None)[1]
         for blk in self.h:
             x = blk(x)
         return self.ln_f(x)
diff --git a/adapcc_b200/ops/gemm.py b/adapcc_b200/ops/gemm.py
--- a/adapcc_b200/ops/gemm.py
+++ b/adapcc_b200/ops/gemm.py
@@ -18,6 +18,7 @@
     if not _bound:
         lib.adapcc_gemm_bias_act_v.argtypes = [c_void_p] * 5 + [c_int] * 5 + [c_void_p]
         lib.adapcc_gemm_pp.argtypes = [c_void_p] * 6 + [c_int] * 4 + [c_void_p]
+        lib.adapcc_transpose_bf16.argtypes = [c_void_p, c_int, c_int, c_void_p, c_void_p]
         _bound = True
     return lib
 
@@ -114,6 +115,7 @@
         y = torch.nn.functional.linear(h, w2, b2)
         ctx.save_for_backward(x, w1, w2, pre, h)
         ctx.params = ((w1, b1), (w2, b2))
+        ctx.fold_bias, ctx.bias_handoff = b2, None
         return y
 
     @staticmethod
@@ -122,8 +124,8 @@
         x, w1, w2, pre, h = ctx.saved_tensors
         p1, p2 = ctx.params
         dy = dy.contiguous()
-        _, dw2, db2 = linear_backward(p2, h, w2, dy, needs_dx=False)
-        w2t = w2.t().contiguous()
+        _, dw2, db2 = linear_backward(p2, h, w2, dy, needs_dx=False, handoff=ctx.bias_handoff)
+        w2t = transpose_bf16(w2)
         if default_variant() == 3 and w2t.shape[0] % 256 == 0:
             db_acc = torch.zeros(w2t.shape[0], dtype=torch.float32, device=dy.device)
             du, _ = linear_act(dy, w2t, None, "dgelu", aux=pre, colsum=db_acc, variant=3)
@@ -134,5 +136,14 @@
         return dx, dw1, db1, dw2, db2
 
 
+def transpose_bf16(a: torch.Tensor) -> torch.Tensor:
+    rows, cols = a.shape
+    out = torch.empty(cols, rows, dtype=a.dtype, device=a.device)
+    if _lib().adapcc_transpose_bf16(c_void_p(a.data_ptr()), rows, cols, c_void_p(out.data_ptr()),
+                                    c_void_p(torch.cuda.current_stream().cuda_stream)) != 0:
+        raise NativeError(f"transpose_bf16 failed: {last_error()}")
+    return out
+
+
 def mlp_gelu(x, w1, b1, w2, b2):
     return _MLPFn.apply(x, w1, b1, w2, b2)
diff --git a/adapcc_b200/ops/layers.py b/adapcc_b200/ops/layers.py
--- a/adapcc_b200/ops/layers.py
+++ b/adapcc_b200/ops/layers.py
@@ -1,6 +1,6 @@
 from __future__ import annotations
 
-from ctypes import c_float, c_int, c_void_p
+from ctypes import c_float, c_int, c_longlong, c_void_p
 
 import torch
 import torch.nn as nn
@@ -21,6 +21,9 @@
         lib.adapcc_ln_bwd.argtypes = [c_void_p] * 9 + [c_int, c_int, c_void_p]
         lib.adapcc_add_ln_fwd.argtypes = [c_void_p] * 8 + [c_int, c_int, c_float, c_void_p]
         lib.adapcc_add_ln_bwd.argtypes = [c_void_p] * 10 + [c_int, c_int, c_void_p]
+        lib.adapcc_add_ln_bwd_bias.argtypes = [c_void_p] * 10 + [c_int, c_void_p, c_int, c_int, c_void_p]
+        lib.adapcc_qkv_pack_colsum.argtypes = [c_void_p] * 4 + [c_int] * 4 + [c_void_p, c_void_p, c_int, c_void_p,
+                                                                             c_void_p]
         lib.adapcc_ln_partials.argtypes = [c_int]
         lib.adapcc_colsum.argtypes = [c_void_p, c_int, c_int, c_void_p, c_void_p, c_void_p]
         lib.adapcc_colsum_splits.argtypes = [c_int]
@@ -88,10 +91,37 @@
     return dgamma, dbeta, finish
 
 
+class _BiasGradHandoff:
+    __slots__ = ("bias", "dy", "db", "in_grad")
+
+    def __init__(self, bias):
+        self.bias, self.dy, self.db, self.in_grad = bias, None, None, False
+
+    def bias_grad_buffer(self, dtype):
+        b = self.bias
+        self.in_grad = _sink(b) is not None and b.grad.dtype == dtype
+        return b.grad if self.in_grad else torch.empty_like(b)
+
+    def set(self, dy, db):
+        self.dy, self.db = dy, db
+
+    def matches(self, dy):
+        return (self.dy is not None and dy.data_ptr() == self.dy.data_ptr() and dy.shape == self.dy.shape
+                and dy.stride() == self.dy.stride())
+
+
+def _fold_bias_grad(out, bias):
+    node = out.grad_fn
+    if bias is None or node is None or getattr(node, "fold_bias", None) is not bias:
+        return None
+    node.bias_handoff = _BiasGradHandoff(bias)
+    return node.bias_handoff
+
+
 class _AddLayerNormFn(torch.autograd.Function):
 
     @staticmethod
-    def forward(ctx, x, res, gamma, beta, eps):
+    def forward(ctx, x, res, gamma, beta, eps, handoff=None):
         lib = _lib()
         d = x.shape[-1]
         x2 = x.reshape(-1, d).contiguous()
@@ -106,6 +136,7 @@
             raise NativeError(f"add_ln_fwd failed: {last_error()}")
         ctx.save_for_backward(ssum, gamma, mean, rstd)
         ctx.params = (gamma, beta)
+        ctx.handoff = handoff
         ctx.set_materialize_grads(False)
         return ssum.view(x.shape), y.view(x.shape)
 
@@ -115,17 +146,64 @@
         s2, gamma, mean, rstd = ctx.saved_tensors
         rows, d = s2.shape
         if dy is None:
-            return dsum, dsum, None, None, None
+            return dsum, dsum, None, None, None, None
         dy2 = dy.reshape(rows, d).contiguous()
         ds2 = None if dsum is None else dsum.reshape(rows, d).contiguous()
+        dres = c_void_p(0) if ds2 is None else _p(ds2)
         dx = torch.empty_like(s2)
         dgamma, dbeta, finish = _ln_param_grads(ctx.params)
-        part = torch.empty(2 * lib.adapcc_ln_partials(rows) * d, dtype=torch.float32, device=s2.device)
-        if lib.adapcc_add_ln_bwd(_p(dy2), _p(s2), _p(gamma), _p(mean), _p(rstd), c_void_p(0) if ds2 is None else _p(ds2),
-                                 _p(dx), _p(dgamma), _p(dbeta), _p(part), rows, d, _s()) != 0:
+        h = ctx.handoff
+        if h is not None:
+            db = h.bias_grad_buffer(dx.dtype)
+            part = torch.empty(3 * lib.adapcc_ln_partials(rows) * d, dtype=torch.float32, device=s2.device)
+            rc = lib.adapcc_add_ln_bwd_bias(_p(dy2), _p(s2), _p(gamma), _p(mean), _p(rstd), dres, _p(dx), _p(dgamma),
+                                            _p(dbeta), _p(db), int(db.dtype == torch.float32), _p(part), rows, d, _s())
+        else:
+            part = torch.empty(2 * lib.adapcc_ln_partials(rows) * d, dtype=torch.float32, device=s2.device)
+            rc = lib.adapcc_add_ln_bwd(_p(dy2), _p(s2), _p(gamma), _p(mean), _p(rstd), dres, _p(dx), _p(dgamma),
+                                       _p(dbeta), _p(part), rows, d, _s())
+        if rc != 0:
             raise NativeError(f"add_ln_bwd failed: {last_error()}")
         dx = dx.view(dy.shape)
-        return (dx, dx) + finish() + (None,)
+        if h is not None:
+            h.set(dx, db)
+        return (dx, dx) + finish() + (None, None)
+
+
+class _QKVSplitFn(torch.autograd.Function):
+
+    @staticmethod
+    def forward(ctx, qkv, n_head, handoff):
+        B, T, D3 = qkv.shape
+        D = D3 // 3
+        ctx.handoff = handoff
+        return tuple(t.view(B, T, n_head, D // n_head).transpose(1, 2) for t in qkv.split(D, dim=-1))
+
+    @staticmethod
+    def backward(ctx, dq, dk, dv):
+        lib = _lib()
+        B, H, T, hd = dq.shape
+        gs = [g if g.stride(-1) == 1 and all(st % 8 == 0 for st in g.stride()[:3]) and g.data_ptr() % 16 == 0
+              else g.contiguous() for g in (dq, dk, dv)]
+        strides = (c_longlong * 9)(*[st for g in gs for st in g.stride()[:3]])
+        dqkv = torch.empty(B, T, 3 * H * hd, dtype=dq.dtype, device=dq.device)
+        h = ctx.handoff
+        db = h.bias_grad_buffer(dq.dtype)
+        part = torch.empty(lib.adapcc_colsum_splits(B * T) * 3 * H * hd, dtype=torch.float32, device=dq.device)
+        if lib.adapcc_qkv_pack_colsum(_p(gs[0]), _p(gs[1]), _p(gs[2]), strides, B, H, T, hd, _p(dqkv), _p(db),
+                                      int(db.dtype == torch.float32), _p(part), _s()) != 0:
+            raise NativeError(f"qkv_pack_colsum failed: {last_error()}")
+        h.set(dqkv, db)
+        return dqkv, None, None
+
+
+def split_heads(qkv, n_head, bias=None):
+    B, T, D3 = qkv.shape
+    handoff = _fold_bias_grad(qkv, bias) if qkv.is_cuda and qkv.dtype == torch.bfloat16 else None
+    if handoff is not None:
+        return _QKVSplitFn.apply(qkv, n_head, handoff)
+    D = D3 // 3
+    return tuple(t.view(B, T, n_head, D // n_head).transpose(1, 2) for t in qkv.split(D, dim=-1))
 
 
 class FusedLayerNorm(nn.LayerNorm):
@@ -139,9 +217,9 @@
             return _LayerNormFn.apply(x, self.weight, self.bias, self.eps)
         return F.layer_norm(x, self.normalized_shape, self.weight, self.bias, self.eps)
 
-    def forward_add(self, x, res):
+    def forward_add(self, x, res, res_bias=None):
         if self._fusable(x) and res.shape == x.shape and res.dtype == x.dtype:
-            return _AddLayerNormFn.apply(x, res, self.weight, self.bias, self.eps)
+            return _AddLayerNormFn.apply(x, res, self.weight, self.bias, self.eps, _fold_bias_grad(res, res_bias))
         s = x + res
         return s, F.layer_norm(s, self.normalized_shape, self.weight, self.bias, self.eps)
 
@@ -151,15 +229,16 @@
     def forward(ctx, x, w, b):
         ctx.save_for_backward(x, w)
         ctx.params = (w, b)
+        ctx.fold_bias, ctx.bias_handoff = b, None
         return F.linear(x, w, b)
 
     @staticmethod
     def backward(ctx, dy):
         x, w = ctx.saved_tensors
-        return linear_backward(ctx.params, x, w, dy, ctx.needs_input_grad[0])
-
-
-def linear_backward(params, x, w, dy, needs_dx=True, db=None):
+        return linear_backward(ctx.params, x, w, dy, ctx.needs_input_grad[0], handoff=ctx.bias_handoff)
+
+
+def linear_backward(params, x, w, dy, needs_dx=True, db=None, handoff=None):
     lib = _lib()
     n = w.shape[0]
     dy2 = dy.reshape(-1, n)
@@ -175,6 +254,12 @@
         dw = None
     else:
         dw = dy2.t() @ x2
+    if handoff is not None and handoff.matches(dy):
+        if handoff.in_grad:
+            sb.begin()
+            sb.done()
+            return dx, dw, None
+        return dx, dw, handoff.db
     rows = dy2.shape[0]
     direct_b = sb is not None and pb.grad.dtype == dy2.dtype and sb.begin()
     if db is not None:
```

Measured after the change: 980,700 tokens/s, median of 6. 1.04x the previous value.
